# ruizhecao96/CMGAN

Hardware: NVIDIA H100
Metric: utterances/sec (2 s @16 kHz) generator fwd+bwd (higher is better)
Workload: dtype tf32

## Files before the change

### cmgan_b200/csrc/ffn_fused.cu

```cuda
#include "common.cuh"
#include "../../include/cmgan_b200.h"
#include "tc_ptx.cuh"

namespace {
using namespace cmgan_tc;

constexpr int BM = 64, C = 64, HID = 256;
constexpr int NT = 128;
constexpr int NCONS = 2, NTHR = NCONS * NT;
constexpr int CHUNK = BM * 128;
constexpr int W_BYTES = 64 * 1024;

__device__ __forceinline__ void consumer_sync(int w) { asm volatile("bar.sync %0, %1;" ::"r"(1 + w), "n"(NT) : "memory"); }

__device__ __forceinline__ uint32_t swz(int r, int c) { return (uint32_t)(r * 128 + ((((c >> 2) ^ r) & 7) << 4) + (c & 3) * 4); }

__device__ __forceinline__ float2 drop_pair(long m, int n, int N, uint32_t seed32, uint32_t thr16, float inv_keep, bool on) {
    if (!on) return make_float2(1.f, 1.f);
    const uint32_t pr = (uint32_t)(((unsigned long long)m * (unsigned long long)N + (unsigned long long)n) >> 1);
    const uint32_t h = cmgan_mix32((pr * 0x9E3779B1u) ^ seed32);
    return make_float2((h & 0xFFFFu) >= thr16 ? inv_keep : 0.f, (h >> 16) >= thr16 ? inv_keep : 0.f);
}

__device__ __forceinline__ void copy_image(uint8_t* dst, const float* src, int bytes) {
    const uint4* s = reinterpret_cast<const uint4*>(src);
    uint4* d = reinterpret_cast<uint4*>(dst);
    for (int i = threadIdx.x; i < bytes / 16; i += NTHR) d[i] = __ldg(s + i);
}

__device__ __forceinline__ float2 ln_tile(const float* __restrict__ x, long ldx, long m0, long M, const float* __restrict__ g,
                                          const float* __restrict__ b, uint8_t* sXn, float* xn_out, int t) {
    const int r = t >> 1, half = t & 1;
    const long m = m0 + r;
    float v[32];
#pragma unroll
    for (int q = 0; q < 8; ++q) {
        float4 t = m < M ? __ldg(reinterpret_cast<const float4*>(x + m * ldx + half * 32 + 4 * q)) : make_float4(0.f, 0.f, 0.f, 0.f);
        v[4 * q] = t.x; v[4 * q + 1] = t.y; v[4 * q + 2] = t.z; v[4 * q + 3] = t.w;
    }
    float s = 0.f;
#pragma unroll
    for (int i = 0; i < 32; ++i) s += v[i];
    s += __shfl_xor_sync(0xffffffffu, s, 1);
    const float mean = s * (1.f / C);
    float q2 = 0.f;
#pragma unroll
    for (int i = 0; i < 32; ++i) { const float d = v[i] - mean; q2 += d * d; }
    q2 += __shfl_xor_sync(0xffffffffu, q2, 1);
    const float rstd = rsqrtf(q2 * (1.f / C) + 1e-5f);
#pragma unroll
    for (int q = 0; q < 8; ++q) {
        float o[4];
#pragma unroll
        for (int j = 0; j < 4; ++j) {
            const int c = half * 32 + 4 * q + j;
            o[j] = m < M ? to_tf32((v[4 * q + j] - mean) * rstd * __ldg(g + c) + __ldg(b + c)) : 0.f;
        }
        *reinterpret_cast<float4*>(sXn + half * CHUNK + swz(r, 4 * q)) = make_float4(o[0], o[1], o[2], o[3]);
        if (xn_out && m < M) *reinterpret_cast<float4*>(xn_out + m * C + half * 32 + 4 * q) = make_float4(o[0], o[1], o[2], o[3]);
    }
    return make_float2(mean, rstd);
}

template <int NB>
__device__ __forceinline__ void mma_chunk64(float (&acc)[4 * NB][8], uint64_t adesc, uint64_t bdesc, bool first) {
#pragma unroll
    for (int k = 0; k < 4; ++k)
#pragma unroll
        for (int b = 0; b < NB; ++b)
            wgmma_m64n64k8_tf32(*reinterpret_cast<float(*)[4][8]>(&acc[4 * b]), adesc + (uint64_t)(2 * k), bdesc + (uint64_t)(512 * b + 2 * k),
                                (first && k == 0) ? 0u : 1u);
}

__device__ __forceinline__ void prefetch_rows_l2(const float* p, long ld, long m0, long M, int t) {
    const long m = m0 + (t >> 1);
    if (m < M) asm volatile("prefetch.global.L2 [%0];" ::"l"(p + m * ld + (t & 1) * 32));
}

struct FfnFwdArgs {
    const float* x; long long ldx; float* out; long long ldo;
    const float* ln_g; const float* ln_b; const float* W1p; const float* b1; const float* W2p; const float* b2;
    long long M; float alpha; unsigned long long seed1, seed2; unsigned int thr; float inv_keep; const unsigned long long* seed_dev;
};

__global__ void __launch_bounds__(NTHR, 1) ffn_fwd_kernel(const __grid_constant__ FfnFwdArgs g) {
    extern __shared__ uint8_t smem_raw[];
    const uint32_t base = (smem_u32(smem_raw) + 1023u) & ~1023u;
    uint8_t* const bp = smem_raw + (base - smem_u32(smem_raw));
    uint8_t* const sW1 = bp;
    uint8_t* const sW2 = bp + W_BYTES;
    const int w = threadIdx.x / NT, t = threadIdx.x % NT;
    const uint32_t xa = base + 2 * W_BYTES + w * 6 * CHUNK, ha = xa + 2 * CHUNK;
    uint8_t* const sXn = bp + (xa - base);
    uint8_t* const sH = bp + (ha - base);
    const int warp = t >> 5, lane = t & 31, fg = lane >> 2, ft = lane & 3;
    const bool drop_on = g.thr != 0u;
    const uint32_t thr16 = g.thr >> 16;
    const uint32_t s1 = cmgan_seed32(cmgan_eff_seed(g.seed1, g.seed_dev)), s2 = cmgan_seed32(cmgan_eff_seed(g.seed2, g.seed_dev));
    copy_image(sW1, g.W1p, W_BYTES);
    copy_image(sW2, g.W2p, W_BYTES);
    fence_proxy_async();
    __syncthreads();
    const long ntiles = (g.M + BM - 1) / BM, stride = (long)NCONS * gridDim.x;
    for (long tile = blockIdx.x + (long)w * gridDim.x; tile < ntiles; tile += stride) {
        const long m0 = tile * BM;
        prefetch_rows_l2(g.x, g.ldx, m0 + stride * BM, g.M, t);
        ln_tile(g.x, g.ldx, m0, g.M, g.ln_g, g.ln_b, sXn, nullptr, t);
        fence_proxy_async();
        consumer_sync(w);
        float acc2[4][8];
#pragma unroll
        for (int hf = 0; hf < 2; ++hf) {
            float acc[8][8];
            wgmma_fence();
            mma_chunk64<2>(acc, gmma_desc_sw128(xa), gmma_desc_sw128(base + hf * 128 * 128), true);
            mma_chunk64<2>(acc, gmma_desc_sw128(xa + CHUNK), gmma_desc_sw128(base + 256 * 128 + hf * 128 * 128), false);
            wgmma_commit();
            wgmma_wait<0>();
            if (hf == 1) consumer_sync(w);
#pragma unroll
            for (int j = 0; j < 8; ++j)
#pragma unroll
                for (int i = 0; i < 2; ++i)
#pragma unroll
                    for (int hh = 0; hh < 2; ++hh) {
                        const int r = 16 * warp + fg + 8 * hh, n = 128 * hf + 16 * j + 8 * i + 2 * ft;
                        const float2 bb = __ldg(reinterpret_cast<const float2*>(g.b1 + n));
                        const float2 ds = drop_pair(m0 + r, n, HID, s1, thr16, g.inv_keep, drop_on);
                        const float h0 = acc[j][4 * i + 2 * hh] + bb.x, h1 = acc[j][4 * i + 2 * hh + 1] + bb.y;
                        *reinterpret_cast<float2*>(sH + ((n >> 5) - 4 * hf) * CHUNK + swz(r, n & 31)) =
                            make_float2(to_tf32(swishf_(h0) * ds.x), to_tf32(swishf_(h1) * ds.y));
                    }
            fence_proxy_async();
            consumer_sync(w);
            wgmma_fence();
#pragma unroll
            for (int c = 0; c < 4; ++c)
                mma_chunk64<1>(acc2, gmma_desc_sw128(ha + c * CHUNK), gmma_desc_sw128(base + W_BYTES + (4 * hf + c) * CHUNK), hf == 0 && c == 0);
            wgmma_commit();
        }
        wgmma_wait<0>();
#pragma unroll
        for (int j = 0; j < 4; ++j)
#pragma unroll
            for (int i = 0; i < 2; ++i)
#pragma unroll
                for (int hh = 0; hh < 2; ++hh) {
                    const long m = m0 + 16 * warp + fg + 8 * hh;
                    if (m >= g.M) continue;
                    const int n = 16 * j + 8 * i + 2 * ft;
                    const float2 bb = __ldg(reinterpret_cast<const float2*>(g.b2 + n));
                    const float2 ds = drop_pair(m, n, C, s2, thr16, g.inv_keep, drop_on);
                    const float2 xr = __ldg(reinterpret_cast<const float2*>(g.x + m * g.ldx + n));
                    *reinterpret_cast<float2*>(g.out + m * g.ldo + n) =
                        make_float2(xr.x + g.alpha * (acc2[j][4 * i + 2 * hh] + bb.x) * ds.x, xr.y + g.alpha * (acc2[j][4 * i + 2 * hh + 1] + bb.y) * ds.y);
                }
    }
}

struct FfnBwdArgs {
    const float* x; long long ldx; const float* dz; long long lddz; const float* dout; long long lddo; const float* res2; long long ldr2;
    const float* ln_g; const float* ln_b; const float* W1p; const float* b1; const float* W2tp; const float* W1tp;
    long long M; unsigned long long seed1; unsigned int thr; float inv_keep; const unsigned long long* seed_dev;
    float* a_out; float* dh_out; float* xn_out; float* stats; float* dx; long long lddx; float* dgamma; float* dbeta;
};

__device__ __forceinline__ void copy_image_kperm(uint8_t* dst, const float* __restrict__ src) {
    for (int u = threadIdx.x; u < W_BYTES / 16; u += NTHR) {
        const int c = u >> 9, n = (u >> 3) & 63, cu = u & 7;
        float v[4];
#pragma unroll
        for (int j = 0; j < 4; ++j) {
            const int k = 8 * (cu >> 1) + 2 * j + (cu & 1);
            v[j] = __ldg(src + c * (CHUNK / 4) + n * 32 + (((k >> 2) ^ (n & 7)) << 2) + (k & 3));
        }
        *reinterpret_cast<float4*>(dst + c * CHUNK + swz(n, 4 * cu)) = make_float4(v[0], v[1], v[2], v[3]);
    }
}

__device__ __forceinline__ void bwd_quarter_mmas(float (&acc)[4][8], float (&dacc)[4][8], const uint32_t (&dzf)[8][4], uint32_t base, uint32_t xa,
                                                 int qt) {
    const uint32_t wrow = (uint32_t)qt * 64 * 128;
    mma_chunk64<1>(acc, gmma_desc_sw128(xa), gmma_desc_sw128(base + wrow), true);
    mma_chunk64<1>(acc, gmma_desc_sw128(xa + CHUNK), gmma_desc_sw128(base + 256 * 128 + wrow), false);
    const uint64_t bdesc = gmma_desc_sw128(base + W_BYTES + wrow);
#pragma unroll
    for (int kk = 0; kk < 8; ++kk)
        wgmma_m64n64k8_tf32_rs(dacc, dzf[kk], bdesc + (uint64_t)((kk >> 2) * (256 * 128 >> 4) + 2 * (kk & 3)), kk > 0 ? 1u : 0u);
}

__global__ void __launch_bounds__(NTHR, 1) ffn_bwd_kernel(const __grid_constant__ FfnBwdArgs g) {
    extern __shared__ uint8_t smem_raw[];
    const uint32_t base = (smem_u32(smem_raw) + 1023u) & ~1023u;
    uint8_t* const bp = smem_raw + (base - smem_u32(smem_raw));
    uint8_t* const sW1 = bp;
    uint8_t* const sW2t = bp + W_BYTES;
    uint8_t* const sW1t = bp + 2 * W_BYTES;
    const int w = threadIdx.x / NT, t = threadIdx.x % NT;
    const uint32_t xa = base + 3 * W_BYTES + w * 2 * CHUNK;
    uint8_t* const sXn = bp + (xa - base);
    float2* const sStats = reinterpret_cast<float2*>(bp + 3 * W_BYTES + NCONS * 2 * CHUNK) + w * BM;
    const int warp = t >> 5, lane = t & 31, fg = lane >> 2, ft = lane & 3;
    const bool drop_on = g.thr != 0u;
    const uint32_t thr16 = g.thr >> 16;
    const uint32_t s1 = cmgan_seed32(cmgan_eff_seed(g.seed1, g.seed_dev));
    copy_image(sW1, g.W1p, W_BYTES);
    copy_image(sW2t, g.W2tp, W_BYTES);
    copy_image_kperm(sW1t, g.W1tp);
    fence_proxy_async();
    __syncthreads();
    float pg[4][4], pb[4][4];
#pragma unroll
    for (int j = 0; j < 4; ++j)
#pragma unroll
        for (int e = 0; e < 4; ++e) pg[j][e] = pb[j][e] = 0.f;
    const long ntiles = (g.M + BM - 1) / BM, stride = (long)NCONS * gridDim.x;
    for (long tile = blockIdx.x + (long)w * gridDim.x; tile < ntiles; tile += stride) {
        const long m0 = tile * BM, mn = m0 + stride * BM;
        prefetch_rows_l2(g.x, g.ldx, mn, g.M, t);
        prefetch_rows_l2(g.dz, g.lddz, mn, g.M, t);
        prefetch_rows_l2(g.dout, g.lddo, mn, g.M, t);
        if (g.res2) prefetch_rows_l2(g.res2, g.ldr2, mn, g.M, t);
        const float2 st = ln_tile(g.x, g.ldx, m0, g.M, g.ln_g, g.ln_b, sXn, g.xn_out, t);
        if ((t & 1) == 0) {
            const long m = m0 + (t >> 1);
            sStats[t >> 1] = st;
            if (m < g.M) reinterpret_cast<float2*>(g.stats)[m] = st;
        }
        uint32_t dzf[8][4];
#pragma unroll
        for (int hh = 0; hh < 2; ++hh) {
            const long m = m0 + 16 * warp + fg + 8 * hh;
#pragma unroll
            for (int kk = 0; kk < 8; ++kk)
#pragma unroll
                for (int e = 0; e < 2; ++e)
                    dzf[kk][hh + 2 * e] = m < g.M ? __float_as_uint(__ldg(g.dz + m * g.lddz + 8 * kk + ft + 4 * e)) : 0u;
        }
        fence_proxy_async();
        consumer_sync(w);
        float acc[4][8], dacc[4][8], dln[4][8];
        wgmma_fence();
        bwd_quarter_mmas(acc, dacc, dzf, base, xa, 0);
        wgmma_commit();
        wgmma_wait<0>();
        uint32_t dha[8][4];
        auto quarter_dh = [&](int qt) {
#pragma unroll
            for (int j = 0; j < 4; ++j)
#pragma unroll
                for (int i = 0; i < 2; ++i)
#pragma unroll
                    for (int hh = 0; hh < 2; ++hh) {
                        const long m = m0 + 16 * warp + fg + 8 * hh;
                        const int n = 64 * qt + 16 * j + 8 * i + 2 * ft;
                        const float2 bb = __ldg(reinterpret_cast<const float2*>(g.b1 + n));
                        const float2 ds = drop_pair(m, n, HID, s1, thr16, g.inv_keep, drop_on);
                        const float h0 = acc[j][4 * i + 2 * hh] + bb.x, h1 = acc[j][4 * i + 2 * hh + 1] + bb.y;
                        const float d0 = to_tf32(dacc[j][4 * i + 2 * hh] * dswishf_(h0) * ds.x);
                        const float d1 = to_tf32(dacc[j][4 * i + 2 * hh + 1] * dswishf_(h1) * ds.y);
                        dha[2 * j + i][hh] = __float_as_uint(d0);
                        dha[2 * j + i][2 + hh] = __float_as_uint(d1);
                        if (m >= g.M) continue;
                        *reinterpret_cast<float2*>(g.a_out + m * HID + n) = make_float2(to_tf32(swishf_(h0) * ds.x), to_tf32(swishf_(h1) * ds.y));
                        *reinterpret_cast<float2*>(g.dh_out + m * HID + n) = make_float2(d0, d1);
                    }
            wgmma_fence();
            const uint64_t bdesc = gmma_desc_sw128(base + 2 * W_BYTES + 2 * qt * CHUNK);
#pragma unroll
            for (int kk = 0; kk < 8; ++kk)
                wgmma_m64n64k8_tf32_rs(dln, dha[kk], bdesc + (uint64_t)((kk >> 2) * (CHUNK >> 4) + 2 * (kk & 3)), (qt > 0 || kk > 0) ? 1u : 0u);
        };
#pragma unroll 1
        for (int qt = 0; qt < 3; ++qt) {
            quarter_dh(qt);
            bwd_quarter_mmas(acc, dacc, dzf, base, xa, qt + 1);
            wgmma_commit();
            wgmma_wait<0>();
        }
        quarter_dh(3);
        wgmma_commit();
        wgmma_wait<0>();
#pragma unroll
        for (int hh = 0; hh < 2; ++hh) {
            const int r = 16 * warp + fg + 8 * hh;
            const long m = m0 + r;
            const bool ok = m < g.M;
            const float2 s = ok ? sStats[r] : make_float2(0.f, 0.f);
            float xh[4][4], dg[4][4], s1r = 0.f, s2r = 0.f;
#pragma unroll
            for (int j = 0; j < 4; ++j)
#pragma unroll
                for (int i = 0; i < 2; ++i) {
                    const int n = 16 * j + 8 * i + 2 * ft;
                    const float2 v = ok ? __ldg(reinterpret_cast<const float2*>(g.x + m * g.ldx + n)) : make_float2(0.f, 0.f);
                    const float2 gm = __ldg(reinterpret_cast<const float2*>(g.ln_g + n));
                    xh[j][2 * i] = (v.x - s.x) * s.y;
                    xh[j][2 * i + 1] = (v.y - s.x) * s.y;
                    dg[j][2 * i] = dln[j][4 * i + 2 * hh] * gm.x;
                    dg[j][2 * i + 1] = dln[j][4 * i + 2 * hh + 1] * gm.y;
                    s1r += dg[j][2 * i] + dg[j][2 * i + 1];
                    s2r += dg[j][2 * i] * xh[j][2 * i] + dg[j][2 * i + 1] * xh[j][2 * i + 1];
                }
            s1r += __shfl_xor_sync(0xffffffffu, s1r, 1);
            s1r += __shfl_xor_sync(0xffffffffu, s1r, 2);
            s2r += __shfl_xor_sync(0xffffffffu, s2r, 1);
            s2r += __shfl_xor_sync(0xffffffffu, s2r, 2);
            const float m1 = s1r * (1.0f / C), m2 = s2r * (1.0f / C);
#pragma unroll
            for (int j = 0; j < 4; ++j)
#pragma unroll
                for (int i = 0; i < 2; ++i) {
                    const int n = 16 * j + 8 * i + 2 * ft;
                    if (ok) {
                        float2 rr = __ldg(reinterpret_cast<const float2*>(g.dout + m * g.lddo + n));
                        if (g.res2) {
                            const float2 r2 = __ldg(reinterpret_cast<const float2*>(g.res2 + m * g.ldr2 + n));
                            rr.x += r2.x; rr.y += r2.y;
                        }
                        *reinterpret_cast<float2*>(g.dx + m * g.lddx + n) =
                            make_float2(s.y * (dg[j][2 * i] - m1 - xh[j][2 * i] * m2) + rr.x, s.y * (dg[j][2 * i + 1] - m1 - xh[j][2 * i + 1] * m2) + rr.y);
                    }
#pragma unroll
                    for (int e = 0; e < 2; ++e) {
                        const float d = dln[j][4 * i + 2 * hh + e];
                        pg[j][2 * i + e] = fmaf(d, xh[j][2 * i + e], pg[j][2 * i + e]);
                        pb[j][2 * i + e] += d;
                    }
                }
        }
        consumer_sync(w);
    }
    float* const red = reinterpret_cast<float*>(bp + 3 * W_BYTES);
    const int cw = threadIdx.x >> 5;
    __syncthreads();
#pragma unroll
    for (int j = 0; j < 4; ++j)
#pragma unroll
        for (int e = 0; e < 4; ++e) {
            float a = pg[j][e], b = pb[j][e];
#pragma unroll
            for (int o = 4; o < 32; o <<= 1) {
                a += __shfl_xor_sync(0xffffffffu, a, o);
                b += __shfl_xor_sync(0xffffffffu, b, o);
            }
            if (fg == 0) {
                const int n = 16 * j + 8 * (e >> 1) + 2 * ft + (e & 1);
                red[cw * 2 * C + n] = a;
                red[cw * 2 * C + C + n] = b;
            }
        }
    __syncthreads();
    if (threadIdx.x < C) {
        const int n = threadIdx.x;
        float v[2][NTHR / 32];
#pragma unroll
        for (int u = 0; u < NTHR / 32; ++u) v[0][u] = red[u * 2 * C + n], v[1][u] = red[u * 2 * C + C + n];
#pragma unroll
        for (int o = 1; o < NTHR / 32; o <<= 1)
#pragma unroll
            for (int u = 0; u < NTHR / 32; u += 2 * o) v[0][u] += v[0][u + o], v[1][u] += v[1][u + o];
        atomicAdd(g.dgamma + n, v[0][0]);
        atomicAdd(g.dbeta + n, v[1][0]);
    }
}

template <typename K>
int prepare(K kernel, size_t smem, const char* name) {
    static bool set = false;
    if (!set) {
        cudaError_t e = cudaFuncSetAttribute(kernel, cudaFuncAttributeMaxDynamicSharedMemorySize, (int)smem);
        if (e != cudaSuccess) { cmgan_set_error("%s: cudaFuncSetAttribute: %s", name, cudaGetErrorString(e)); return -1; }
        set = true;
    }
    return 0;
}

}

CMGAN_API int cmgan_ffn_fwd(const float* x, long long ldx, long long M, const float* ln_g, const float* ln_b, const float* W1p, const float* b1,
                            const float* W2p, const float* b2, float alpha, unsigned long long seed1, unsigned long long seed2, unsigned int thr,
                            float inv_keep, const unsigned long long* seed_dev, float* out, long long ldo, void* stream) {
    CMGAN_REQUIRE(x && out && ln_g && ln_b && W1p && b1 && W2p && b2 && M >= 0 && ldx % 4 == 0 && ldo % 2 == 0, "cmgan_ffn_fwd: bad arguments");
    if (M == 0) return 0;
    const size_t smem = 1024 + 2 * W_BYTES + NCONS * (2 * CHUNK + 4 * CHUNK);
    if (prepare(ffn_fwd_kernel, smem, "ffn_fwd_kernel")) return -1;
    FfnFwdArgs a{x, ldx, out, ldo, ln_g, ln_b, W1p, b1, W2p, b2, M, alpha, seed1, seed2, thr, inv_keep, seed_dev};
    const long ntiles = (M + BM - 1) / BM, half_tiles = (ntiles + 1) / 2;
    const int grid = (int)(half_tiles < cmgan_num_sms() ? half_tiles : cmgan_num_sms());
    ffn_fwd_kernel<<<grid, NTHR, smem, (cudaStream_t)stream>>>(a);
    return cmgan_check_launch("ffn_fwd_kernel");
}

CMGAN_API int cmgan_ffn_bwd(const float* x, long long ldx, const float* dz, long long lddz, const float* dout, long long lddo, const float* res2,
                            long long ldr2, long long M, const float* ln_g, const float* ln_b, const float* W1p, const float* b1, const float* W2tp,
                            const float* W1tp, unsigned long long seed1, unsigned int thr, float inv_keep, const unsigned long long* seed_dev,
                            float* dx, long long lddx, float* a_out, float* dh_out, float* xn_out, float* dgamma, float* dbeta, float* ws,
                            void* stream) {
    CMGAN_REQUIRE(x && dz && dout && ln_g && ln_b && W1p && b1 && W2tp && W1tp && dx && a_out && dh_out && xn_out && dgamma && dbeta && ws && M >= 0 &&
                  ldx % 4 == 0 && lddz % 4 == 0, "cmgan_ffn_bwd: bad arguments");
    CMGAN_REQUIRE(lddo % 2 == 0 && (!res2 || ldr2 % 2 == 0) && lddx % 2 == 0, "cmgan_ffn_bwd: bad arguments");
    if (M == 0) return 0;
    const size_t smem = 1024 + 3 * W_BYTES + NCONS * (2 * CHUNK + BM * sizeof(float2));
    if (prepare(ffn_bwd_kernel, smem, "ffn_bwd_kernel")) return -1;
    float* stats = ws + C * M;
    FfnBwdArgs a{x, ldx, dz, lddz, dout, lddo, res2, res2 ? ldr2 : 0, ln_g, ln_b, W1p, b1, W2tp, W1tp, M, seed1, thr, inv_keep, seed_dev,
                 a_out, dh_out, xn_out, stats, dx, lddx, dgamma, dbeta};
    const long ntiles = (M + BM - 1) / BM, half_tiles = (ntiles + 1) / 2;
    const int grid = (int)(half_tiles < cmgan_num_sms() ? half_tiles : cmgan_num_sms());
    ffn_bwd_kernel<<<grid, NTHR, smem, (cudaStream_t)stream>>>(a);
    return cmgan_check_launch("ffn_bwd_kernel");
}
```

Before: 97.41.

## Pipeline FFN forward in quarter chunks with three consumer warpgroups

```diff
diff --git a/cmgan_b200/csrc/ffn_fused.cu b/cmgan_b200/csrc/ffn_fused.cu
--- a/cmgan_b200/csrc/ffn_fused.cu
+++ b/cmgan_b200/csrc/ffn_fused.cu
@@ -22,10 +22,11 @@
     return make_float2((h & 0xFFFFu) >= thr16 ? inv_keep : 0.f, (h >> 16) >= thr16 ? inv_keep : 0.f);
 }
 
+template <int THREADS = NTHR>
 __device__ __forceinline__ void copy_image(uint8_t* dst, const float* src, int bytes) {
     const uint4* s = reinterpret_cast<const uint4*>(src);
     uint4* d = reinterpret_cast<uint4*>(dst);
-    for (int i = threadIdx.x; i < bytes / 16; i += NTHR) d[i] = __ldg(s + i);
+    for (int i = threadIdx.x; i < bytes / 16; i += THREADS) d[i] = __ldg(s + i);
 }
 
 __device__ __forceinline__ float2 ln_tile(const float* __restrict__ x, long ldx, long m0, long M, const float* __restrict__ g,
@@ -83,60 +84,68 @@
     long long M; float alpha; unsigned long long seed1, seed2; unsigned int thr; float inv_keep; const unsigned long long* seed_dev;
 };
 
-__global__ void __launch_bounds__(NTHR, 1) ffn_fwd_kernel(const __grid_constant__ FfnFwdArgs g) {
+constexpr int NCONS_FWD = 3, NTHR_FWD = NCONS_FWD * NT;
+
+__global__ void __launch_bounds__(NTHR_FWD, 1) ffn_fwd_kernel(const __grid_constant__ FfnFwdArgs g) {
     extern __shared__ uint8_t smem_raw[];
     const uint32_t base = (smem_u32(smem_raw) + 1023u) & ~1023u;
     uint8_t* const bp = smem_raw + (base - smem_u32(smem_raw));
     uint8_t* const sW1 = bp;
     uint8_t* const sW2 = bp + W_BYTES;
     const int w = threadIdx.x / NT, t = threadIdx.x % NT;
-    const uint32_t xa = base + 2 * W_BYTES + w * 6 * CHUNK, ha = xa + 2 * CHUNK;
+    const uint32_t xa = base + 2 * W_BYTES + w * 4 * CHUNK, ha = xa + 2 * CHUNK;
     uint8_t* const sXn = bp + (xa - base);
     uint8_t* const sH = bp + (ha - base);
     const int warp = t >> 5, lane = t & 31, fg = lane >> 2, ft = lane & 3;
     const bool drop_on = g.thr != 0u;
     const uint32_t thr16 = g.thr >> 16;
     const uint32_t s1 = cmgan_seed32(cmgan_eff_seed(g.seed1, g.seed_dev)), s2 = cmgan_seed32(cmgan_eff_seed(g.seed2, g.seed_dev));
-    copy_image(sW1, g.W1p, W_BYTES);
-    copy_image(sW2, g.W2p, W_BYTES);
+    copy_image<NTHR_FWD>(sW1, g.W1p, W_BYTES);
+    copy_image<NTHR_FWD>(sW2, g.W2p, W_BYTES);
     fence_proxy_async();
     __syncthreads();
-    const long ntiles = (g.M + BM - 1) / BM, stride = (long)NCONS * gridDim.x;
-    for (long tile = blockIdx.x + (long)w * gridDim.x; tile < ntiles; tile += stride) {
+    const long ntiles = (g.M + BM - 1) / BM, stride = (long)NCONS_FWD * gridDim.x;
+    long tile = blockIdx.x + (long)w * gridDim.x;
+    if (tile < ntiles) {
+        prefetch_rows_l2(g.x, g.ldx, tile * BM + stride * BM, g.M, t);
+        ln_tile(g.x, g.ldx, tile * BM, g.M, g.ln_g, g.ln_b, sXn, nullptr, t);
+    }
+    for (; tile < ntiles; tile += stride) {
         const long m0 = tile * BM;
-        prefetch_rows_l2(g.x, g.ldx, m0 + stride * BM, g.M, t);
-        ln_tile(g.x, g.ldx, m0, g.M, g.ln_g, g.ln_b, sXn, nullptr, t);
         fence_proxy_async();
         consumer_sync(w);
-        float acc2[4][8];
-#pragma unroll
-        for (int hf = 0; hf < 2; ++hf) {
-            float acc[8][8];
-            wgmma_fence();
-            mma_chunk64<2>(acc, gmma_desc_sw128(xa), gmma_desc_sw128(base + hf * 128 * 128), true);
-            mma_chunk64<2>(acc, gmma_desc_sw128(xa + CHUNK), gmma_desc_sw128(base + 256 * 128 + hf * 128 * 128), false);
-            wgmma_commit();
+        float acc[4][8], acc2[4][8];
+        wgmma_fence();
+        mma_chunk64<1>(acc, gmma_desc_sw128(xa), gmma_desc_sw128(base), true);
+        mma_chunk64<1>(acc, gmma_desc_sw128(xa + CHUNK), gmma_desc_sw128(base + 256 * 128), false);
+        wgmma_commit();
+#pragma unroll
+        for (int q = 0; q < 4; ++q) {
             wgmma_wait<0>();
-            if (hf == 1) consumer_sync(w);
-#pragma unroll
-            for (int j = 0; j < 8; ++j)
+            if (q > 0) consumer_sync(w);
+#pragma unroll
+            for (int j = 0; j < 4; ++j)
 #pragma unroll
                 for (int i = 0; i < 2; ++i)
 #pragma unroll
                     for (int hh = 0; hh < 2; ++hh) {
-                        const int r = 16 * warp + fg + 8 * hh, n = 128 * hf + 16 * j + 8 * i + 2 * ft;
+                        const int r = 16 * warp + fg + 8 * hh, n = 64 * q + 16 * j + 8 * i + 2 * ft;
                         const float2 bb = __ldg(reinterpret_cast<const float2*>(g.b1 + n));
                         const float2 ds = drop_pair(m0 + r, n, HID, s1, thr16, g.inv_keep, drop_on);
                         const float h0 = acc[j][4 * i + 2 * hh] + bb.x, h1 = acc[j][4 * i + 2 * hh + 1] + bb.y;
-                        *reinterpret_cast<float2*>(sH + ((n >> 5) - 4 * hf) * CHUNK + swz(r, n & 31)) =
+                        *reinterpret_cast<float2*>(sH + ((n >> 5) & 1) * CHUNK + swz(r, n & 31)) =
                             make_float2(to_tf32(swishf_(h0) * ds.x), to_tf32(swishf_(h1) * ds.y));
                     }
             fence_proxy_async();
             consumer_sync(w);
             wgmma_fence();
 #pragma unroll
-            for (int c = 0; c < 4; ++c)
-                mma_chunk64<1>(acc2, gmma_desc_sw128(ha + c * CHUNK), gmma_desc_sw128(base + W_BYTES + (4 * hf + c) * CHUNK), hf == 0 && c == 0);
+            for (int c = 0; c < 2; ++c)
+                mma_chunk64<1>(acc2, gmma_desc_sw128(ha + c * CHUNK), gmma_desc_sw128(base + W_BYTES + (2 * q + c) * CHUNK), q == 0 && c == 0);
+            if (q < 3) {
+                mma_chunk64<1>(acc, gmma_desc_sw128(xa), gmma_desc_sw128(base + (q + 1) * 64 * 128), true);
+                mma_chunk64<1>(acc, gmma_desc_sw128(xa + CHUNK), gmma_desc_sw128(base + 256 * 128 + (q + 1) * 64 * 128), false);
+            }
             wgmma_commit();
         }
         wgmma_wait<0>();
@@ -155,6 +164,10 @@
                     *reinterpret_cast<float2*>(g.out + m * g.ldo + n) =
                         make_float2(xr.x + g.alpha * (acc2[j][4 * i + 2 * hh] + bb.x) * ds.x, xr.y + g.alpha * (acc2[j][4 * i + 2 * hh + 1] + bb.y) * ds.y);
                 }
+        if (tile + stride < ntiles) {
+            prefetch_rows_l2(g.x, g.ldx, m0 + 2 * stride * BM, g.M, t);
+            ln_tile(g.x, g.ldx, m0 + stride * BM, g.M, g.ln_g, g.ln_b, sXn, nullptr, t);
+        }
     }
 }
 
@@ -280,6 +293,24 @@
         }
         quarter_dh(3);
         wgmma_commit();
+        float2 xv[2][4][2], rr[2][4][2];
+#pragma unroll
+        for (int hh = 0; hh < 2; ++hh) {
+            const long m = m0 + 16 * warp + fg + 8 * hh;
+            const bool ok = m < g.M;
+#pragma unroll
+            for (int j = 0; j < 4; ++j)
+#pragma unroll
+                for (int i = 0; i < 2; ++i) {
+                    const int n = 16 * j + 8 * i + 2 * ft;
+                    xv[hh][j][i] = ok ? __ldg(reinterpret_cast<const float2*>(g.x + m * g.ldx + n)) : make_float2(0.f, 0.f);
+                    rr[hh][j][i] = ok ? __ldg(reinterpret_cast<const float2*>(g.dout + m * g.lddo + n)) : make_float2(0.f, 0.f);
+                    if (ok && g.res2) {
+                        const float2 r2 = __ldg(reinterpret_cast<const float2*>(g.res2 + m * g.ldr2 + n));
+                        rr[hh][j][i].x += r2.x; rr[hh][j][i].y += r2.y;
+                    }
+                }
+        }
         wgmma_wait<0>();
 #pragma unroll
         for (int hh = 0; hh < 2; ++hh) {
@@ -293,7 +324,7 @@
 #pragma unroll
                 for (int i = 0; i < 2; ++i) {
                     const int n = 16 * j + 8 * i + 2 * ft;
-                    const float2 v = ok ? __ldg(reinterpret_cast<const float2*>(g.x + m * g.ldx + n)) : make_float2(0.f, 0.f);
+                    const float2 v = xv[hh][j][i];
                     const float2 gm = __ldg(reinterpret_cast<const float2*>(g.ln_g + n));
                     xh[j][2 * i] = (v.x - s.x) * s.y;
                     xh[j][2 * i + 1] = (v.y - s.x) * s.y;
@@ -312,15 +343,9 @@
 #pragma unroll
                 for (int i = 0; i < 2; ++i) {
                     const int n = 16 * j + 8 * i + 2 * ft;
-                    if (ok) {
-                        float2 rr = __ldg(reinterpret_cast<const float2*>(g.dout + m * g.lddo + n));
-                        if (g.res2) {
-                            const float2 r2 = __ldg(reinterpret_cast<const float2*>(g.res2 + m * g.ldr2 + n));
-                            rr.x += r2.x; rr.y += r2.y;
-                        }
-                        *reinterpret_cast<float2*>(g.dx + m * g.lddx + n) =
-                            make_float2(s.y * (dg[j][2 * i] - m1 - xh[j][2 * i] * m2) + rr.x, s.y * (dg[j][2 * i + 1] - m1 - xh[j][2 * i + 1] * m2) + rr.y);
-                    }
+                    if (ok)
+                        *reinterpret_cast<float2*>(g.dx + m * g.lddx + n) = make_float2(s.y * (dg[j][2 * i] - m1 - xh[j][2 * i] * m2) + rr[hh][j][i].x,
+                                                                                        s.y * (dg[j][2 * i + 1] - m1 - xh[j][2 * i + 1] * m2) + rr[hh][j][i].y);
 #pragma unroll
                     for (int e = 0; e < 2; ++e) {
                         const float d = dln[j][4 * i + 2 * hh + e];
@@ -383,12 +408,12 @@
                             float inv_keep, const unsigned long long* seed_dev, float* out, long long ldo, void* stream) {
     CMGAN_REQUIRE(x && out && ln_g && ln_b && W1p && b1 && W2p && b2 && M >= 0 && ldx % 4 == 0 && ldo % 2 == 0, "cmgan_ffn_fwd: bad arguments");
     if (M == 0) return 0;
-    const size_t smem = 1024 + 2 * W_BYTES + NCONS * (2 * CHUNK + 4 * CHUNK);
+    const size_t smem = 1024 + 2 * W_BYTES + NCONS_FWD * (2 * CHUNK + 2 * CHUNK);
     if (prepare(ffn_fwd_kernel, smem, "ffn_fwd_kernel")) return -1;
     FfnFwdArgs a{x, ldx, out, ldo, ln_g, ln_b, W1p, b1, W2p, b2, M, alpha, seed1, seed2, thr, inv_keep, seed_dev};
-    const long ntiles = (M + BM - 1) / BM, half_tiles = (ntiles + 1) / 2;
-    const int grid = (int)(half_tiles < cmgan_num_sms() ? half_tiles : cmgan_num_sms());
-    ffn_fwd_kernel<<<grid, NTHR, smem, (cudaStream_t)stream>>>(a);
+    const long ntiles = (M + BM - 1) / BM, pass_tiles = (ntiles + NCONS_FWD - 1) / NCONS_FWD;
+    const int grid = (int)(pass_tiles < cmgan_num_sms() ? pass_tiles : cmgan_num_sms());
+    ffn_fwd_kernel<<<grid, NTHR_FWD, smem, (cudaStream_t)stream>>>(a);
     return cmgan_check_launch("ffn_fwd_kernel");
 }
 
```

Result: no change. 98.37, median of 6 (+1.0%).
